# IceLab-X/FidelityFusion

Measured on AMD Instinct MI355X. Metric: GP NLML+Cholesky throughput (NxN fp64 GF/s, %MFMA-roofline) at N=16384, higher is better.
Workload: dtype f64; 1 GPU; headline: single-fidelity cigp NLML forward, ARD kernel, 1 block of N=16384 D=16 d=1 (BASELINE configs[2]); N=16384, D=16, d=1, blocks=1, blocks_in_flight_per_rank=1, parallelism=fidelity-shard x1 (LPT partition, one 8-byte all-reduce per step)

## Files before the change

### fidelityfusion_amd/csrc/gemm.hip

```cpp
#include <algorithm>

#include "ffgp_internal.h"

#define BK 16
#ifndef FFGP_PD_SMALL
#define FFGP_PD_SMALL 4
#endif

#ifdef FFGP_GEMM_TRACE
__device__ unsigned long long* ffgp_trace_buf = nullptr;
extern "C" int ffgp_debug_set_trace(void* p) {
  return hipMemcpyToSymbol(HIP_SYMBOL(ffgp_trace_buf), &p, sizeof(p)) == hipSuccess ? 0 : -1;
}
#define FFGP_TRACE(slot)                                                                            \
  do {                                                                                              \
    if (tid == 0 && ffgp_trace_buf) {                                                               \
      ffgp_trace_buf[(size_t)bid * 8 + (slot)] = __builtin_readcyclecounter();                      \
      if ((slot) == 0) {                                                                            \
        unsigned hwid = 0, xcc = 0;                                                                 \
        asm volatile("s_getreg_b32 %0, hwreg(HW_REG_HW_ID)" : "=s"(hwid));                          \
        asm volatile("s_getreg_b32 %0, hwreg(HW_REG_XCC_ID)" : "=s"(xcc));                          \
        ffgp_trace_buf[(size_t)bid * 8 + 6] = ((unsigned long long)xcc << 32) | hwid;               \
        ffgp_trace_buf[(size_t)bid * 8 + 7] = wall_clock64();                                       \
      }                                                                                             \
    }                                                                                               \
  } while (0)
#else
#define FFGP_TRACE(slot)
#endif

template <int TS>
struct Geo {
  static constexpr int WT = TS / 32;
  static constexpr int NLD = TS / 32;
  static constexpr int MNLD = TS + 16;
  static constexpr int OPBUF = 16 * (TS + 16);
};

__device__ __forceinline__ d2_t ld2_guard(const double* p, int rem, bool vec) {
  d2_t v = {0.0, 0.0};
  if (rem >= 2) {
    if (vec) {
      v = *reinterpret_cast<const d2_t*>(p);
    } else {
      v.x = p[0];
      v.y = p[1];
    }
  } else if (rem == 1) {
    v.x = p[0];
  }
  return v;
}

template <int OP, int TS, bool GUARD>
__device__ __forceinline__ void gload(const double* __restrict__ P, int ld, int r0, int R, int k0, int K, int tid,
                                      bool vec, d2_t (&v)[Geo<TS>::NLD]) {
#pragma unroll
  for (int i = 0; i < Geo<TS>::NLD; ++i) {
    const int idx = tid + 256 * i;
    d2_t z = {0.0, 0.0};
    if (OP == OP_KMAJOR) {
      const int row = idx >> 3, ch = idx & 7;
      const int gr = r0 + row, gk = k0 + ch * 2;
      if (GUARD)
        v[i] = (gr < R) ? ld2_guard(P + (size_t)gr * ld + gk, K - gk, vec) : z;
      else
        v[i] = *reinterpret_cast<const d2_t*>(P + (size_t)gr * ld + gk);
    } else {
      const int kk = idx / (TS / 2), c2 = idx % (TS / 2);
      const int gk = k0 + kk, gr = r0 + c2 * 2;
      if (GUARD)
        v[i] = (gk < K) ? ld2_guard(P + (size_t)gk * ld + gr, R - gr, vec) : z;
      else
        v[i] = *reinterpret_cast<const d2_t*>(P + (size_t)gk * ld + gr);
    }
  }
}

template <int OP, int TS>
__device__ __forceinline__ void sstore(double* s, int tid, const d2_t (&v)[Geo<TS>::NLD]) {
#pragma unroll
  for (int i = 0; i < Geo<TS>::NLD; ++i) {
    const int idx = tid + 256 * i;
    if (OP == OP_KMAJOR) {
      const int row = idx >> 3, ch = idx & 7;
      *reinterpret_cast<d2_t*>(s + row * 16 + ((ch ^ ((row >> 1) & 7)) << 1)) = v[i];
    } else {
      const int kk = idx / (TS / 2), c2 = idx % (TS / 2);
      *reinterpret_cast<d2_t*>(s + kk * Geo<TS>::MNLD + c2 * 2) = v[i];
    }
  }
}

template <int OP, int TS>
__device__ __forceinline__ void frag_offsets(int lane, int wbase, int (&off)[4]) {
#pragma unroll
  for (int kq = 0; kq < 4; ++kq) {
    if (OP == OP_KMAJOR) {
      const int row = wbase + (lane & 15);
      const int c0 = (lane >> 5) ^ ((lane & 15) >> 1);
      off[kq] = row * 16 + ((((kq << 1) ^ c0)) << 1) + ((lane >> 4) & 1);
    } else {
      off[kq] = (kq * 4 + (lane >> 4)) * Geo<TS>::MNLD + wbase + (lane & 15);
    }
  }
}

__device__ __forceinline__ void decode_tile(int t, int mode, int tiles_m, int tiles_n, int& ti, int& tj, const int GL = 3) {
  const int G = 1 << GL;
  if (mode == TILES_FULL) {
    const int band_sz = G * tiles_n;
    int r0 = 0;
    while (t >= band_sz) {
      t -= band_sz;
      r0 += G;
    }
    const int hgt = min(G, tiles_m - r0);
    if (hgt == G) {
      tj = t >> GL;
      ti = r0 + (t & (G - 1));
    } else {
      tj = t / hgt;
      ti = r0 + t % hgt;
    }
  } else {
    int r0 = 0, hgt = 0, fc = 0;
    while (true) {
      hgt = min(G, tiles_m - r0);
      fc = min(r0, tiles_n);
      const int nc = max(0, min(hgt, tiles_n - r0));
      const int cnt = hgt * fc + nc * hgt - nc * (nc - 1) / 2;
      if (t < cnt) break;
      t -= cnt;
      r0 += hgt;
    }
    if (t < hgt * fc) {
      if (hgt == G) {
        tj = t >> GL;
        ti = r0 + (t & (G - 1));
      } else {
        tj = t / hgt;
        ti = r0 + t % hgt;
      }
    } else {
      t -= hgt * fc;
      int c = 0;
      while (t >= hgt - c) {
        t -= hgt - c;
        ++c;
      }
      tj = r0 + c;
      ti = r0 + c + t;
    }
  }
}

template <int OP, int TS>
__device__ __forceinline__ void lane_byte_offsets(int ld, int tid, unsigned (&voff)[Geo<TS>::NLD]) {
#pragma unroll
  for (int i = 0; i < Geo<TS>::NLD; ++i) {
    const int idx = tid + 256 * i;
    if (OP == OP_KMAJOR) {
      const int row = idx >> 3, ch = idx & 7;
      voff[i] = (unsigned)(row * ld + ch * 2) * 8u;
    } else {
      const int kk = idx / (TS / 2), c2 = idx % (TS / 2);
      voff[i] = (unsigned)(kk * ld + c2 * 2) * 8u;
    }
  }
}

template <int TS>
__device__ __forceinline__ void gload_fast(const char* __restrict__ base, const unsigned (&voff)[Geo<TS>::NLD],
                                           d2_t (&v)[Geo<TS>::NLD]) {
#pragma unroll
  for (int i = 0; i < Geo<TS>::NLD; ++i) v[i] = *reinterpret_cast<const d2_t*>(base + voff[i]);
}

template <int OP, int TS>
constexpr int opbuf() { return OP == OP_KMAJOR ? TS * 16 : Geo<TS>::OPBUF; }

template <int OPA, int OPB, int TM, int TN, bool NEG, int PD>
__device__ __forceinline__ void gemm_tile_fast(const char* __restrict__ baseA, const char* __restrict__ baseB, size_t stepA,
                                               size_t stepB, char* __restrict__ baseC, size_t row4_bytes, unsigned voffC,
                                               bool load_c, double* smem, int nkt, int tid,
                                               const unsigned (&voffA)[Geo<TM>::NLD], const unsigned (&voffB)[Geo<TN>::NLD],
                                               const int (&offA)[4], const int (&offB)[4], int trace_bid) {
  constexpr int WM = Geo<TM>::WT, WN = Geo<TN>::WT;
  constexpr int BUFA = opbuf<OPA, TM>(), BUFB = opbuf<OPB, TN>(), STAGE = BUFA + BUFB;
  constexpr int subA = (OPA == OP_KMAJOR) ? 256 : 16;
  constexpr int subB = (OPB == OP_KMAJOR) ? 256 : 16;
  static_assert(PD == 1 || (PD & 1) == 0, "prefetch depth must be 1 or even (LDS stage parity is compile-time)");
  d2_t ra[PD][Geo<TM>::NLD], rb[PD][Geo<TN>::NLD];
#pragma unroll
  for (int s = 0; s < PD; ++s) {
    if (s < nkt) {
      gload_fast<TM>(baseA + s * stepA, voffA, ra[s]);
      gload_fast<TN>(baseB + s * stepB, voffB, rb[s]);
    }
  }
  d4_t acc[WM][WN];
  if (load_c) {
#pragma unroll
    for (int i = 0; i < WM; ++i)
#pragma unroll
      for (int r = 0; r < 4; ++r) {
        const char* rowb = baseC + (size_t)(i * 4 + r) * row4_bytes;
#pragma unroll
        for (int j = 0; j < WN; ++j) acc[i][j][r] = *reinterpret_cast<const double*>(rowb + voffC + j * 128);
      }
  } else {
#pragma unroll
    for (int i = 0; i < WM; ++i)
#pragma unroll
      for (int j = 0; j < WN; ++j) acc[i][j] = (d4_t){0.0, 0.0, 0.0, 0.0};
  }
  sstore<OPA, TM>(smem, tid, ra[0]);
  sstore<OPB, TN>(smem + BUFA, tid, rb[0]);
  __syncthreads();
#ifdef FFGP_GEMM_TRACE
  if (tid == 0 && ffgp_trace_buf) ffgp_trace_buf[(size_t)trace_bid * 8 + 1] = __builtin_readcyclecounter();
#endif
  baseA += (size_t)PD * stepA;
  baseB += (size_t)PD * stepB;
  for (int kt0 = 0; kt0 < nkt; kt0 += PD) {
#pragma unroll
    for (int u = 0; u < PD; ++u) {
      const int kt = kt0 + u;
      if (kt >= nkt) break;
      const int par = (PD == 1) ? (kt & 1) : (u & 1);
      const double* sA = smem + par * STAGE;
      const double* sB = sA + BUFA;
      if (kt + PD < nkt) {
        gload_fast<TM>(baseA, voffA, ra[u]);
        gload_fast<TN>(baseB, voffB, rb[u]);
        baseA += stepA;
        baseB += stepB;
      }
#pragma unroll
      for (int kq = 0; kq < 4; ++kq) {
        double a[WM], b[WN];
#pragma unroll
        for (int i = 0; i < WM; ++i) a[i] = sA[offA[kq] + i * subA];
#pragma unroll
        for (int j = 0; j < WN; ++j) b[j] = sB[offB[kq] + j * subB];
#pragma unroll
        for (int i = 0; i < WM; ++i)
#pragma unroll
          for (int j = 0; j < WN; ++j)
            acc[i][j] = __builtin_amdgcn_mfma_f64_16x16x4f64(a[i], b[j], acc[i][j], 0, 0, NEG ? 1 : 0);
      }
      if (kt + 1 < nkt) {
        double* dA = smem + (par ^ 1) * STAGE;
        sstore<OPA, TM>(dA, tid, ra[(u + 1) % PD]);
        sstore<OPB, TN>(dA + BUFA, tid, rb[(u + 1) % PD]);
      }
      __syncthreads();
    }
  }
#ifdef FFGP_GEMM_TRACE
  if (tid == 0 && ffgp_trace_buf) ffgp_trace_buf[(size_t)trace_bid * 8 + 2] = __builtin_readcyclecounter();
#endif
#pragma unroll
  for (int i = 0; i < WM; ++i)
#pragma unroll
    for (int r = 0; r < 4; ++r) {
      char* rowb = baseC + (size_t)(i * 4 + r) * row4_bytes;
#pragma unroll
      for (int j = 0; j < WN; ++j) *reinterpret_cast<double*>(rowb + voffC + j * 128) = acc[i][j][r];
    }
}

template <int OPA, int OPB, int TM, int TN, bool GUARD>
__device__ __forceinline__ void gemm_mainloop(const GemmArgs& p, const double* __restrict__ Ag, const double* __restrict__ Bg,
                                              double* smem, int m0, int n0, int kt0, int kt1, int tid,
                                              const int (&offA)[4], const int (&offB)[4],
                                              d4_t (&acc)[Geo<TM>::WT][Geo<TN>::WT]) {
  constexpr int WM = Geo<TM>::WT, WN = Geo<TN>::WT;
  constexpr int BUFA = opbuf<OPA, TM>(), BUFB = opbuf<OPB, TN>(), STAGE = BUFA + BUFB;
  constexpr int subA = (OPA == OP_KMAJOR) ? 256 : 16;
  constexpr int subB = (OPB == OP_KMAJOR) ? 256 : 16;
  d2_t ra[Geo<TM>::NLD], rb[Geo<TN>::NLD];
  gload<OPA, TM, GUARD>(Ag, p.lda, m0, p.m, kt0 * BK, p.k, tid, p.avec != 0, ra);
  gload<OPB, TN, GUARD>(Bg, p.ldb, n0, p.n, kt0 * BK, p.k, tid, p.bvec != 0, rb);
  sstore<OPA, TM>(smem, tid, ra);
  sstore<OPB, TN>(smem + BUFA, tid, rb);
  __syncthreads();
  for (int kt = kt0; kt < kt1; ++kt) {
    const int par = (kt - kt0) & 1;
    const double* sA = smem + par * STAGE;
    const double* sB = sA + BUFA;
    const bool more = (kt + 1 < kt1);
    if (more) {
      gload<OPA, TM, GUARD>(Ag, p.lda, m0, p.m, (kt + 1) * BK, p.k, tid, p.avec != 0, ra);
      gload<OPB, TN, GUARD>(Bg, p.ldb, n0, p.n, (kt + 1) * BK, p.k, tid, p.bvec != 0, rb);
    }
#pragma unroll
    for (int kq = 0; kq < 4; ++kq) {
      double a[WM], b[WN];
#pragma unroll
      for (int i = 0; i < WM; ++i) a[i] = sA[offA[kq] + i * subA];
#pragma unroll
      for (int j = 0; j < WN; ++j) b[j] = sB[offB[kq] + j * subB];
#pragma unroll
      for (int i = 0; i < WM; ++i)
#pragma unroll
        for (int j = 0; j < WN; ++j) acc[i][j] = __builtin_amdgcn_mfma_f64_16x16x4f64(a[i], b[j], acc[i][j], 0, 0, 0);
    }
    if (more) {
      double* dA = smem + (par ^ 1) * STAGE;
      sstore<OPA, TM>(dA, tid, ra);
      sstore<OPB, TN>(dA + BUFA, tid, rb);
    }
    __syncthreads();
  }
}

template <int OPA, int OPB, int MODE, int TM, int TN>
__device__ __forceinline__ void gemm_one_tile(const GemmArgs& p, const double* __restrict__ Ag, const double* __restrict__ Bg,
                                              double* __restrict__ Cg, double* smem, int ti, int tj, const int tid, const int bid) {
  constexpr int WM = Geo<TM>::WT, WN = Geo<TN>::WT;
  const int lane = tid & 63, wave = tid >> 6;
  const int wm = wave >> 1, wn = wave & 1;
  int offA[4], offB[4];
  frag_offsets<OPA, TM>(lane, wm * (TM / 2), offA);
  frag_offsets<OPB, TN>(lane, wn * (TN / 2), offB);
  const bool fast_ab = p.fast && p.avec && p.bvec;
  const int m0 = ti * TM, n0 = tj * TN;

  int kbeg = 0, kend = p.k;
  if (p.lo_i) kbeg = max(kbeg, ti * TM);
  if (p.lo_j) kbeg = max(kbeg, tj * TN);
  if (p.hi_i) kend = min(kend, (ti + 1) * TM);
  if (p.hi_j) kend = min(kend, (tj + 1) * TN);
  const int kt0 = kbeg / BK;
  const int kt1 = (kend + BK - 1) / BK;

  const bool interior = (m0 + TM <= p.m) && (n0 + TN <= p.n) && (kt1 * BK <= p.k) && p.avec && p.bvec;
  if constexpr (TM == 128 && TN == 128 && OPA == OP_KMAJOR && OPB == OP_KMAJOR) {
    if (p.pack && fast_ab && interior && kt0 == 0 && kt1 * BK == p.k && !(MODE == TILES_LOWER && m0 < n0 + TN)) return;
  }
  if (fast_ab && interior && kt0 < kt1 && !(MODE == TILES_LOWER && m0 < n0 + TN)) {
    const size_t k0 = (size_t)kt0 * BK;
    const char* bA = reinterpret_cast<const char*>(Ag) +
                     ((OPA == OP_KMAJOR) ? ((size_t)m0 * p.lda + k0) : (k0 * p.lda + m0)) * 8;
    const char* bB = reinterpret_cast<const char*>(Bg) +
                     ((OPB == OP_KMAJOR) ? ((size_t)n0 * p.ldb + k0) : (k0 * p.ldb + n0)) * 8;
    const size_t stepA = (OPA == OP_KMAJOR) ? (size_t)BK * 8 : (size_t)BK * p.lda * 8;
    const size_t stepB = (OPB == OP_KMAJOR) ? (size_t)BK * 8 : (size_t)BK * p.ldb * 8;
    char* bC = reinterpret_cast<char*>(Cg) + ((size_t)m0 * p.ldc + n0) * 8;
    const size_t row4 = (size_t)p.ldc * 32;
    constexpr int PD = (TM == 128) ? 1 : FFGP_PD_SMALL;
    unsigned voffA[Geo<TM>::NLD], voffB[Geo<TN>::NLD];
    lane_byte_offsets<OPA, TM>(p.lda, tid, voffA);
    lane_byte_offsets<OPB, TN>(p.ldb, tid, voffB);
    const unsigned voffC = (unsigned)((wm * (TM / 2) + (lane >> 4)) * p.ldc + wn * (TN / 2) + (lane & 15)) * 8u;
    if (p.alpha < 0.0)
      gemm_tile_fast<OPA, OPB, TM, TN, true, PD>(bA, bB, stepA, stepB, bC, row4, voffC, p.beta != 0.0, smem, kt1 - kt0, tid, voffA,
                                             voffB, offA, offB, bid);
    else
      gemm_tile_fast<OPA, OPB, TM, TN, false, PD>(bA, bB, stepA, stepB, bC, row4, voffC, p.beta != 0.0, smem, kt1 - kt0, tid, voffA,
                                              voffB, offA, offB, bid);
    FFGP_TRACE(3);
    return;
  }

  d4_t acc[WM][WN];
#pragma unroll
  for (int i = 0; i < WM; ++i)
#pragma unroll
    for (int j = 0; j < WN; ++j) acc[i][j] = (d4_t){0.0, 0.0, 0.0, 0.0};

  if (kt0 < kt1) {
    if (interior)
      gemm_mainloop<OPA, OPB, TM, TN, false>(p, Ag, Bg, smem, m0, n0, kt0, kt1, tid, offA, offB, acc);
    else
      gemm_mainloop<OPA, OPB, TM, TN, true>(p, Ag, Bg, smem, m0, n0, kt0, kt1, tid, offA, offB, acc);
  }

  FFGP_TRACE(2);
  const double alpha = p.alpha, beta = p.beta;
  const bool use_c = (beta != 0.0);
  const int rbase0 = m0 + wm * (TM / 2) + (lane >> 4);
  const int cbase = n0 + wn * (TN / 2) + (lane & 15);
  double cv[2][4][WN];
  auto load_group = [&](int i, double (&dst)[4][WN]) {
#pragma unroll
    for (int r = 0; r < 4; ++r) {
      const int rowc = min(rbase0 + i * 16 + 4 * r, p.m - 1);
#pragma unroll
      for (int j = 0; j < WN; ++j) {
        const int colc = min(cbase + j * 16, p.n - 1);
        dst[r][j] = Cg[(size_t)rowc * p.ldc + colc];
      }
    }
  };
  if (use_c) {
    load_group(0, cv[0]);
  } else {
#pragma unroll
    for (int b = 0; b < 2; ++b)
#pragma unroll
      for (int r = 0; r < 4; ++r)
#pragma unroll
        for (int j = 0; j < WN; ++j) cv[b][r][j] = 0.0;
  }
#pragma unroll
  for (int i = 0; i < WM; ++i) {
    if (use_c && i + 1 < WM) load_group(i + 1, cv[(i + 1) & 1]);
#pragma unroll
    for (int r = 0; r < 4; ++r) {
      const int row = rbase0 + i * 16 + 4 * r;
#pragma unroll
      for (int j = 0; j < WN; ++j) {
        const int col = cbase + j * 16;
        if (row < p.m && col < p.n && (MODE != TILES_LOWER || col <= row)) {
          Cg[(size_t)row * p.ldc + col] = alpha * acc[i][j][r] + beta * cv[i & 1][r][j];
        }
      }
    }
  }
  FFGP_TRACE(3);
}

template <int OPA, int OPB, int MODE, int TM, int TN>
__device__ __forceinline__ void gemm_block(const GemmArgs& p, const double* __restrict__ Ag, const double* __restrict__ Bg,
                                           double* __restrict__ Cg, double* smem, const int tid, const int bid) {
  FFGP_TRACE(0);
  if constexpr (TM == 128 && TN == 128) {
    if (bid >= p.split_at) {
      const int q = bid - p.split_at;
      int Ti, Tj;
      decode_tile(p.split_at + (q >> 2), MODE, p.tiles_m, p.tiles_n, Ti, Tj, p.band_log2);
      const int ti = __builtin_amdgcn_readfirstlane(2 * Ti + ((q >> 1) & 1));
      const int tj = __builtin_amdgcn_readfirstlane(2 * Tj + (q & 1));
      if (ti * 64 >= p.m || tj * 64 >= p.n || (MODE == TILES_LOWER && tj > ti)) return;
      gemm_one_tile<OPA, OPB, MODE, 64, 64>(p, Ag, Bg, Cg, smem, ti, tj, tid, bid);
      return;
    }
  }
  int t = bid;
  if (!(p.lo_i | p.lo_j | p.hi_i | p.hi_j)) {
    const int nwg = p.total_tiles;
    const int q = nwg >> 3, r = nwg & 7, xcd = bid & 7;
    t = (xcd < r ? xcd * (q + 1) : r * (q + 1) + (xcd - r) * q) + (bid >> 3);
  }
  int ti, tj;
  decode_tile(t, MODE, p.tiles_m, p.tiles_n, ti, tj, p.band_log2);
  ti = __builtin_amdgcn_readfirstlane(ti);
  tj = __builtin_amdgcn_readfirstlane(tj);
  gemm_one_tile<OPA, OPB, MODE, TM, TN>(p, Ag, Bg, Cg, smem, ti, tj, tid, bid);
}

template <int OPA, int OPB, int MODE, int TAG, int TM, int TN>
__global__ __launch_bounds__(256, 2) void ffgp_gemm_f64(GemmArgs p) {
  __shared__ __attribute__((aligned(16))) double smem[2 * (opbuf<OPA, TM>() + opbuf<OPB, TN>())];
  const int tid = threadIdx.x;
  if (p.pub_word && tid == 0 && blockIdx.x == 0 && blockIdx.y == 0 && blockIdx.z == 0)
    __hip_atomic_store(p.pub_word, p.pub_val, __ATOMIC_RELAXED, __HIP_MEMORY_SCOPE_SYSTEM);
  if (p.prio) __builtin_amdgcn_s_setprio(2);
  const double* __restrict__ Ag = p.A + (size_t)blockIdx.y * p.sA + (size_t)blockIdx.z * p.sA2;
  const double* __restrict__ Bg = p.B + (size_t)blockIdx.y * p.sB + (size_t)blockIdx.z * p.sB2;
  double* __restrict__ Cg = p.C + (size_t)blockIdx.y * p.sC + (size_t)blockIdx.z * p.sC2;
  gemm_block<OPA, OPB, MODE, TM, TN>(p, Ag, Bg, Cg, smem, tid, blockIdx.x);
}

template <int OPA, int OPB, int MODE, int TAG, int TM, int TN>
__global__ __launch_bounds__(256, 2) void ffgp_gemm_f64_rag(GemmRag q) {
  __shared__ __attribute__((aligned(16))) double smem[2 * (opbuf<OPA, TM>() + opbuf<OPB, TN>())];
  const int tid = threadIdx.x;
  const GemmRagMember& r = q.mem[blockIdx.y];
  if ((int)blockIdx.x >= r.grid) return;
  if (q.base.prio) __builtin_amdgcn_s_setprio(2);
  GemmArgs p = q.base;
  p.A = r.A; p.B = r.B; p.C = r.C;
  p.m = r.m; p.n = r.n; p.k = r.k;
  p.lda = r.lda; p.ldb = r.ldb; p.ldc = r.ldc;
  p.tiles_m = r.tiles_m; p.tiles_n = r.tiles_n; p.total_tiles = r.total_tiles;
  p.grid = r.grid; p.split_at = r.split_at;
  p.fast = r.fast; p.avec = r.avec; p.bvec = r.bvec;
  gemm_block<OPA, OPB, MODE, TM, TN>(p, p.A, p.B, p.C, smem, tid, blockIdx.x);
}

#define GEMM_BAND_LOG2 3
#define POLITE_PAD_KB 40
template <int OPA, int OPB, int MODE, int TAG, int TM, int TN>
static int launch_t(ffgp_handle* h, const GemmArgs& a) {
  if (a.pad_lds > 0)
    FFGP_HIP(hipFuncSetAttribute(reinterpret_cast<const void*>(&ffgp_gemm_f64<OPA, OPB, MODE, TAG, TM, TN>),
                                 hipFuncAttributeMaxDynamicSharedMemorySize, 64 * 1024));
  hipLaunchKernelGGL((ffgp_gemm_f64<OPA, OPB, MODE, TAG, TM, TN>), dim3(a.grid, a.batch, a.batch2), dim3(256), a.pad_lds, h->stream, a);
  return FFGP_OK;
}

template <int TS>
static int dispatch(ffgp_handle* h, int opa, int opb, int mode, int syrk_tag, const GemmArgs& a) {
  if (syrk_tag) {
    if (opa == OP_KMAJOR && opb == OP_KMAJOR && mode == TILES_LOWER) return launch_t<OP_KMAJOR, OP_KMAJOR, TILES_LOWER, 1, TS, TS>(h, a);
  } else if (mode == TILES_LOWER) {
    if (opa == OP_KMAJOR && opb == OP_KMAJOR) return launch_t<OP_KMAJOR, OP_KMAJOR, TILES_LOWER, 0, TS, TS>(h, a);
    if (opa == OP_MNMAJOR && opb == OP_MNMAJOR) return launch_t<OP_MNMAJOR, OP_MNMAJOR, TILES_LOWER, 0, TS, TS>(h, a);
  } else {
    if (opa == OP_KMAJOR && opb == OP_KMAJOR) return launch_t<OP_KMAJOR, OP_KMAJOR, TILES_FULL, 0, TS, TS>(h, a);
    if (opa == OP_KMAJOR && opb == OP_MNMAJOR) return launch_t<OP_KMAJOR, OP_MNMAJOR, TILES_FULL, 0, TS, TS>(h, a);
    if (opa == OP_MNMAJOR && opb == OP_MNMAJOR) return launch_t<OP_MNMAJOR, OP_MNMAJOR, TILES_FULL, 0, TS, TS>(h, a);
    if (opa == OP_MNMAJOR && opb == OP_KMAJOR) return launch_t<OP_MNMAJOR, OP_KMAJOR, TILES_FULL, 0, TS, TS>(h, a);
  }
  return FFGP_ERR_ARG;
}

static inline bool aligned16(const void* p) { return (reinterpret_cast<uintptr_t>(p) & 15) == 0; }

static int count_tiles(int mode, int m, int n, int tsm, int tsn, int& tm, int& tn) {
  tm = (m + tsm - 1) / tsm;
  tn = (n + tsn - 1) / tsn;
  if (mode != TILES_LOWER) return tm * tn;
  int total = 0;
  for (int ti = 0; ti < tm; ++ti) total += (ti + 1 < tn) ? ti + 1 : tn;
  return total;
}

__global__ __launch_bounds__(256) void ffgp_splitk_reduce(const double* __restrict__ P, int ldp, long sP, int parts, double* __restrict__ C,
                                                         int ldc, int m, int n, double beta) {
  const long e = (long)blockIdx.x * 256 + threadIdx.x;
  if (e >= (long)m * n) return;
  const int r = (int)(e / n), c = (int)(e - (long)r * n);
  double acc = 0.0;
  const double* p = P + (size_t)r * ldp + c;
  for (int s = 0; s < parts; ++s) acc += p[(size_t)s * sP];
  double* dst = C + (size_t)r * ldc + c;
  *dst = (beta != 0.0) ? acc + beta * *dst : acc;
}

static int ensure_skw(ffgp_handle* h, size_t bytes) {
  if (bytes <= h->skw_bytes) return FFGP_OK;
  if (h->skw) {
    hipStreamSynchronize(h->stream);
    if (h->aux) hipStreamSynchronize(h->aux);
    hipFree(h->skw);
  }
  h->skw = nullptr;
  h->skw_bytes = 0;
  const size_t gran = (size_t)16 << 20;
  const size_t want = (bytes + gran - 1) / gran * gran;
  if (hipMalloc(&h->skw, want) != hipSuccess) return FFGP_ERR_ALLOC;
  h->skw_bytes = want;
  ++h->alloc_epoch;
  return FFGP_OK;
}

struct SkinnyArgs {
  const double* A;
  const double* B;
  double* C;
  int m, n, k, lda, ldb, ldc, opb;
  int kc;
  long sP;
  int klo;
  int ldcj;
  double alpha, beta;
};

__device__ __forceinline__ double skinny_b(const SkinnyArgs& p, int kk, int j) {
  return (p.opb == OP_KMAJOR) ? p.B[(size_t)j * p.ldb + kk] : p.B[(size_t)kk * p.ldb + j];
}

template <int NC>
__global__ __launch_bounds__(256) void ffgp_skinny_kmajor(SkinnyArgs p) {
  const int lane = threadIdx.x & 63;
  const int row = blockIdx.x * 4 + (threadIdx.x >> 6);
  if (row >= p.m) return;
  const double* __restrict__ a = p.A + (size_t)row * p.lda;
  const int kbeg = blockIdx.y * p.kc, kend = min(p.k, kbeg + p.kc);
  double acc[NC];
#pragma unroll
  for (int j = 0; j < NC; ++j) acc[j] = 0.0;
#pragma unroll 4
  for (int k0 = max(kbeg, p.klo ? (row & ~127) : 0) + lane * 2; k0 < kend; k0 += 128) {
    const double a0 = a[k0];
    const bool two = k0 + 1 < kend;
    const double a1 = two ? a[k0 + 1] : 0.0;
#pragma unroll
    for (int j = 0; j < NC; ++j)
      if (j < p.n) {
        acc[j] = __builtin_fma(a0, skinny_b(p, k0, j), acc[j]);
        if (two) acc[j] = __builtin_fma(a1, skinny_b(p, k0 + 1, j), acc[j]);
      }
  }
#pragma unroll
  for (int j = 0; j < NC; ++j)
    for (int o = 32; o > 0; o >>= 1) acc[j] += __shfl_down(acc[j], o);
  if (lane == 0) {
#pragma unroll
    for (int j = 0; j < NC; ++j)
      if (j < p.n) {
        double* dst = p.C + blockIdx.y * p.sP + (size_t)row * p.ldc + (size_t)j * p.ldcj;
        *dst = (p.beta != 0.0) ? p.alpha * acc[j] + p.beta * *dst : p.alpha * acc[j];
      }
  }
}

template <int NC>
__global__ __launch_bounds__(512) void ffgp_skinny_mnmajor(SkinnyArgs p) {
  __shared__ double red[8][NC][64];
  const int lane = threadIdx.x & 63, w = threadIdx.x >> 6;
  const int row = blockIdx.x * 64 + lane;
  const int kbeg = blockIdx.y * p.kc, kend = min(p.k, kbeg + p.kc);
  const int k00 = max(kbeg, p.klo ? (int)blockIdx.x * 64 : 0);
  const int kchunk = (max(kend - k00, 0) + 7) / 8;
  const int kb = k00 + w * kchunk, ke = min(kend, kb + kchunk);
  double acc[NC];
#pragma unroll
  for (int j = 0; j < NC; ++j) acc[j] = 0.0;
  if (row < p.m) {
    const double* __restrict__ a = p.A + row;
#pragma unroll 8
    for (int kk = kb; kk < ke; ++kk) {
      const double av = a[(size_t)kk * p.lda];
#pragma unroll
      for (int j = 0; j < NC; ++j)
        if (j < p.n) acc[j] = __builtin_fma(av, skinny_b(p, kk, j), acc[j]);
    }
  }
#pragma unroll
  for (int j = 0; j < NC; ++j) red[w][j][lane] = acc[j];
  __syncthreads();
  if (w == 0 && row < p.m) {
#pragma unroll
    for (int j = 0; j < NC; ++j)
      if (j < p.n) {
        double s = 0.0;
#pragma unroll
        for (int q = 0; q < 8; ++q) s += red[q][j][lane];
        double* dst = p.C + blockIdx.y * p.sP + (size_t)row * p.ldc + (size_t)j * p.ldcj;
        *dst = (p.beta != 0.0) ? p.alpha * s + p.beta * *dst : p.alpha * s;
      }
  }
}

template <int NC>
static void launch_skinny(ffgp_handle* h, int opa, const SkinnyArgs& a, int parts = 1) {
  if (opa == OP_KMAJOR)
    hipLaunchKernelGGL(ffgp_skinny_kmajor<NC>, dim3((a.m + 3) / 4, parts), dim3(256), 0, h->stream, a);
  else
    hipLaunchKernelGGL(ffgp_skinny_mnmajor<NC>, dim3((a.m + 63) / 64, parts), dim3(512), 0, h->stream, a);
}

struct GemmPlan {
  GemmArgs a;
  int tsm, tsn;
  int syrk_tag;
};

static int gemm_plan(ffgp_handle* h, int opa, int opb, int mode, int syrk_tag, const double* A, int lda, const double* B, int ldb, double* C,
                     int ldc, int m, int n, int k, double alpha, double beta, int tri, int alias, int batch, long sA, long sB, long sC,
                     GemmPlan& pl) {
  GemmArgs& a = pl.a;
  a = GemmArgs();
  a.avec = (!(lda & 1) && aligned16(A)) ? 1 : 0;
  a.bvec = (!(ldb & 1) && aligned16(B)) ? 1 : 0;
  a.A = A; a.B = B; a.C = C;
  a.m = m; a.n = n; a.k = k;
  a.lda = lda; a.ldb = ldb; a.ldc = ldc;
  a.alpha = alpha; a.beta = beta;
  a.prio = (h->stream == h->aux && h->aux_prio) ? 1 : 0;
  a.batch2 = 1;
  a.sA2 = a.sB2 = a.sC2 = 0;
  const int dec_batch = (batch < 0) ? 1 : (batch > 1 ? batch : 1);
  if (batch < 0) batch = -batch;
  a.batch = batch > 1 ? batch : 1;
  a.sA = sA; a.sB = sB; a.sC = sC;
  if ((sA & 1) || (sB & 1)) a.avec = a.bvec = 0;
  a.lo_i = (tri & TRI_LO_I) ? 1 : 0;
  a.lo_j = (tri & TRI_LO_J) ? 1 : 0;
  a.hi_i = (tri & TRI_HI_I) ? 1 : 0;
  a.hi_j = (tri & TRI_HI_J) ? 1 : 0;
  int tsm = 128, tsn = 128;
  a.total_tiles = count_tiles(mode, m, n, 128, 128, a.tiles_m, a.tiles_n);
  int level = 0;
  if (h->force_ts == 64) level = 1;
  else if (h->force_ts == 32) level = 2;
  else if (h->force_ts == 0 && a.total_tiles * dec_batch < h->small_tile_threshold) level = 1;
  const bool kk = (opa == OP_KMAJOR && opb == OP_KMAJOR);
  if (level >= 1) {
    if (alias == 0 || (alias == ALIAS_A && n <= 64) || (alias == ALIAS_B && m <= 64)) {
      tsm = tsn = 64;
    } else if (alias == ALIAS_A && kk) {
      tsm = 64;
    }
    a.total_tiles = count_tiles(mode, m, n, tsm, tsn, a.tiles_m, a.tiles_n);
    if (h->force_ts == 0 && level == 1 && kk && dec_batch == 1 && tsm == 64 && a.total_tiles < h->tile32_threshold) level = 2;
    if (level == 2 && kk && tsm == 64 && dec_batch == 1 && alias != ALIAS_B) {
      tsm = 32;
      tsn = (alias == ALIAS_A) ? 128 : 32;
      a.total_tiles = count_tiles(mode, m, n, tsm, tsn, a.tiles_m, a.tiles_n);
    }
  }
  if ((alias == ALIAS_A && a.tiles_n != 1) || (alias == ALIAS_B && a.tiles_m != 1)) {
    fprintf(stderr, "[ffgp] gemm: in-place launch would be split across %d x %d tiles (alias %d)\n", a.tiles_m, a.tiles_n, alias);
    return FFGP_ERR_ARG;
  }
  a.fast = ((alpha == 1.0 || alpha == -1.0) && (beta == 0.0 || beta == 1.0) && (size_t)lda * 8 * 130 < 0xffffffffull &&
            (size_t)ldb * 8 * 130 < 0xffffffffull && (size_t)ldc * 8 * 130 < 0xffffffffull)
               ? 1 : 0;
  a.grid = a.total_tiles;
  a.split_at = 0x7fffffff;
  a.band_log2 = GEMM_BAND_LOG2;
  if (tsm == 128 && tsn == 128 && alias == 0 && dec_batch == 1 && h->force_ts == 0 && h->split_rem_max > 0 && a.total_tiles > 256) {
    const int rem = a.total_tiles % 256;
    if (rem > 0 && rem <= h->split_rem_max) {
      a.split_at = a.total_tiles - rem;
      a.total_tiles = a.split_at;
      a.grid = a.split_at + 4 * rem;
    }
  }
  a.pad_lds = 0;
  if (syrk_tag && tsm == 128 && h->lookahead && h->polite_m > 0 && m < h->polite_m && h->stream != h->aux) a.pad_lds = POLITE_PAD_KB * 1024;
  if (syrk_tag && tsm == 64 && tsn == 64 && h->polite64_active && h->polite64_pad_kb > 0 && h->stream != h->aux && dec_batch == 1 &&
      m - n <= 1024)
    a.pad_lds = h->polite64_pad_kb * 1024;
  if (syrk_tag && tsm == 32 && tsn == 32 && h->polite64_active && h->polite32_pad_kb > 0 && h->stream != h->aux && dec_batch == 1 && m - n <= 1024)
    a.pad_lds = h->polite32_pad_kb * 1024;
  a.pub_word = nullptr;
  a.pub_val = 0;
  if (h->ho_gdefer_slot >= 0 && h->ho_gdefer_stream == h->stream && h->ob_F <= 1) {
    a.pub_word = h->ho_mem + h->ho_gdefer_slot * 16;
    a.pub_val = h->ho_seq[h->ho_gdefer_slot];
    h->ho_launched[h->ho_gdefer_slot] = h->ho_seq[h->ho_gdefer_slot];
    h->ho_gdefer_slot = -1;
  }
  if (tsm != 128) syrk_tag = 0;
  pl.tsm = tsm; pl.tsn = tsn; pl.syrk_tag = syrk_tag;
  return FFGP_OK;
}

int ffgp_gemm_launch(ffgp_handle* h, int opa, int opb, int mode, int syrk_tag, const double* A, int lda, const double* B,
                     int ldb, double* C, int ldc, int m, int n, int k, double alpha, double beta, int tri, int alias, int batch,
                     long sA, long sB, long sC) {
  if (m <= 0 || n <= 0) return FFGP_OK;
  if (k <= 0) {
    return FFGP_ERR_ARG;
  }
  if (!A || !B || !C) return FFGP_ERR_ARG;
  if (mode == TILES_LOWER && m < n) return FFGP_ERR_ARG;
  if (alias == ALIAS_A && (n > 128 || mode != TILES_FULL)) return FFGP_ERR_ARG;
  if (alias == ALIAS_B && (m > 128 || mode != TILES_FULL)) return FFGP_ERR_ARG;
  const bool ob = h->ob_F > 1;
  long ob_sA = 0, ob_sB = 0, ob_sC = 0;
  if (ob) {
    auto stride_of = [&](const double* ptr, long& st) {
      for (int i = 0; i < h->ob_n; ++i)
        if (ptr >= h->ob_rng[i].lo && ptr < h->ob_rng[i].hi) { st = h->ob_rng[i].stride; return true; }
      return false;
    };
    if (!stride_of(A, ob_sA) || !stride_of(B, ob_sB) || !stride_of(C, ob_sC) || ((ob_sA | ob_sB | ob_sC) & 1) || alias != 0 || syrk_tag) {
      fprintf(stderr, "[ffgp] gemm: outer-batch launch with an operand outside the registered ranges\n");
      return FFGP_ERR_ARG;
    }
    if (tri == 0 || m <= 8 || n <= 8) {
      const int F = h->ob_F;
      h->ob_F = 0;
      int rc = FFGP_OK;
      for (int f = 0; f < F && rc == FFGP_OK; ++f)
        rc = ffgp_gemm_launch(h, opa, opb, mode, syrk_tag, A + (size_t)f * ob_sA, lda, B + (size_t)f * ob_sB, ldb, C + (size_t)f * ob_sC, ldc,
                              m, n, k, alpha, beta, tri, alias, batch, sA, sB, sC);
      h->ob_F = F;
      return rc;
    }
  }
  if (h->skinny_max_n > 0 && m <= h->skinny_max_n && m <= 8 && n > 8 && alias == 0 && (batch == 0 || batch == 1) && (tri == 0 || tri == TRI_LO_J) &&
      mode == TILES_FULL && !syrk_tag && h->stream != h->aux) {
// ... 262 lines not shown
```

Before: 52440 GF/s.

## Software-pipeline LDS fragment reads and split MFMA batches around global loads in GEMM

Restructures the fast GEMM tile main loop so the next k-quarter's LDS fragments are read ahead into double-buffered registers while the current MFMAs issue. The LDS store and the next global prefetch move into the middle of the MFMA stream, and only one barrier per k-tile remains, implemented as an explicit waitcnt plus s_barrier. The aim is to hide LDS and global-memory latency behind MFMA work. Separately, 32x32 tiles now get a higher minimum-workgroups launch bound (6), which raises occupancy at the cost of register pressure. Per-k-tile cycle tracing is also added, but only under the trace build flag.

```diff
diff --git a/fidelityfusion_amd/csrc/gemm.hip b/fidelityfusion_amd/csrc/gemm.hip
--- a/fidelityfusion_amd/csrc/gemm.hip
+++ b/fidelityfusion_amd/csrc/gemm.hip
@@ -12,9 +12,15 @@
 extern "C" int ffgp_debug_set_trace(void* p) {
   return hipMemcpyToSymbol(HIP_SYMBOL(ffgp_trace_buf), &p, sizeof(p)) == hipSuccess ? 0 : -1;
 }
+__device__ unsigned* ffgp_trace_seq = nullptr;
+__device__ unsigned ffgp_trace_cap = 0;
+extern "C" int ffgp_debug_set_trace_seq(void* counter, unsigned cap) {
+  return hipMemcpyToSymbol(HIP_SYMBOL(ffgp_trace_cap), &cap, sizeof(cap)) == hipSuccess &&
+                 hipMemcpyToSymbol(HIP_SYMBOL(ffgp_trace_seq), &counter, sizeof(counter)) == hipSuccess ? 0 : -1;
+}
 #define FFGP_TRACE(slot)                                                                            \
   do {                                                                                              \
-    if (tid == 0 && ffgp_trace_buf) {                                                               \
+    if (tid == 0 && ffgp_trace_buf && !ffgp_trace_seq) {                                            \
       ffgp_trace_buf[(size_t)bid * 8 + (slot)] = __builtin_readcyclecounter();                      \
       if ((slot) == 0) {                                                                            \
         unsigned hwid = 0, xcc = 0;                                                                 \
@@ -25,8 +31,17 @@
       }                                                                                             \
     }                                                                                               \
   } while (0)
+#define KT_STAMP(v)                          \
+  do {                                       \
+    if (KT_TRACE) {                          \
+      __builtin_amdgcn_sched_barrier(0);     \
+      v = __builtin_readcyclecounter();      \
+      __builtin_amdgcn_sched_barrier(0);     \
+    }                                        \
+  } while (0)
 #else
 #define FFGP_TRACE(slot)
+#define KT_STAMP(v)
 #endif
 
 template <int TS>
@@ -180,6 +195,22 @@
 template <int OP, int TS>
 constexpr int opbuf() { return OP == OP_KMAJOR ? TS * 16 : Geo<TS>::OPBUF; }
 
+#define GEMM_LDS_WAIT()                      \
+  do {                                       \
+    __builtin_amdgcn_sched_barrier(0);       \
+    asm volatile("" ::: "memory");           \
+    __builtin_amdgcn_s_waitcnt(0xc07f);      \
+  } while (0)
+#define GEMM_BARRIER() asm volatile("s_barrier" ::: "memory")
+
+template <int WM, int WN, int subA, int subB>
+__device__ __forceinline__ void frag_read(const double* sA, const double* sB, int oa, int ob, double (&a)[WM], double (&b)[WN]) {
+#pragma unroll
+  for (int i = 0; i < WM; ++i) a[i] = sA[oa + i * subA];
+#pragma unroll
+  for (int j = 0; j < WN; ++j) b[j] = sB[ob + j * subB];
+}
+
 template <int OPA, int OPB, int TM, int TN, bool NEG, int PD>
 __device__ __forceinline__ void gemm_tile_fast(const char* __restrict__ baseA, const char* __restrict__ baseB, size_t stepA,
                                                size_t stepB, char* __restrict__ baseC, size_t row4_bytes, unsigned voffC,
@@ -191,6 +222,9 @@
   constexpr int subA = (OPA == OP_KMAJOR) ? 256 : 16;
   constexpr int subB = (OPB == OP_KMAJOR) ? 256 : 16;
   static_assert(PD == 1 || (PD & 1) == 0, "prefetch depth must be 1 or even (LDS stage parity is compile-time)");
+  constexpr bool AHEAD = !(TM == 32 && TN == 128);
+  constexpr int HALF = (WM * WN + 1) / 2;
+  constexpr int U = (PD == 1) ? 2 : PD;
   d2_t ra[PD][Geo<TM>::NLD], rb[PD][Geo<TN>::NLD];
 #pragma unroll
   for (int s = 0; s < PD; ++s) {
@@ -199,6 +233,8 @@
       gload_fast<TN>(baseB + s * stepB, voffB, rb[s]);
     }
   }
+  baseA += (size_t)PD * stepA;
+  baseB += (size_t)PD * stepB;
   d4_t acc[WM][WN];
   if (load_c) {
 #pragma unroll
@@ -217,49 +253,109 @@
   }
   sstore<OPA, TM>(smem, tid, ra[0]);
   sstore<OPB, TN>(smem + BUFA, tid, rb[0]);
-  __syncthreads();
+  if (PD < nkt) {
+    gload_fast<TM>(baseA, voffA, ra[0]);
+    gload_fast<TN>(baseB, voffB, rb[0]);
+    baseA += stepA;
+    baseB += stepB;
+  }
+  GEMM_LDS_WAIT();
+  GEMM_BARRIER();
+  double fa[2][WM], fb[2][WN];
+  if (AHEAD) frag_read<WM, WN, subA, subB>(smem, smem + BUFA, offA[0], offB[0], fa[0], fb[0]);
 #ifdef FFGP_GEMM_TRACE
-  if (tid == 0 && ffgp_trace_buf) ffgp_trace_buf[(size_t)trace_bid * 8 + 1] = __builtin_readcyclecounter();
+  constexpr bool KT_TRACE = (TM == 128 && TN == 128);
+  size_t trow = (size_t)trace_bid;
+  bool ton = (tid == 0 && ffgp_trace_buf);
+  if (ton && ffgp_trace_seq) {
+    ton = false;
+    if (KT_TRACE) {
+      const unsigned r = atomicAdd(ffgp_trace_seq, 1u);
+      if (r < ffgp_trace_cap) {
+        unsigned hwid = 0, xcc = 0;
+        asm volatile("s_getreg_b32 %0, hwreg(HW_REG_HW_ID)" : "=s"(hwid));
+        asm volatile("s_getreg_b32 %0, hwreg(HW_REG_XCC_ID)" : "=s"(xcc));
+        ton = true;
+        trow = r;
+        ffgp_trace_buf[trow * 8 + 6] = ((unsigned long long)gridDim.x << 40) | ((unsigned long long)(xcc & 0xf) << 32) | hwid;
+        ffgp_trace_buf[trow * 8 + 7] = wall_clock64();
+      }
+    }
+  }
+  if (ton) ffgp_trace_buf[trow * 8 + 1] = __builtin_readcyclecounter();
+  unsigned long long t_l = 0, t_b = 0, t_x = 0, t_m = 0, t_w0 = 0, t_w1 = 0;
+  unsigned kt_first = 0, kt_vm = 0, kt_bar = 0, kt_lds = 0;
 #endif
-  baseA += (size_t)PD * stepA;
-  baseB += (size_t)PD * stepB;
-  for (int kt0 = 0; kt0 < nkt; kt0 += PD) {
-#pragma unroll
-    for (int u = 0; u < PD; ++u) {
+  for (int kt0 = 0; kt0 < nkt; kt0 += U) {
+#pragma unroll
+    for (int u = 0; u < U; ++u) {
       const int kt = kt0 + u;
       if (kt >= nkt) break;
-      const int par = (PD == 1) ? (kt & 1) : (u & 1);
-      const double* sA = smem + par * STAGE;
-      const double* sB = sA + BUFA;
-      if (kt + PD < nkt) {
-        gload_fast<TM>(baseA, voffA, ra[u]);
-        gload_fast<TN>(baseB, voffB, rb[u]);
-        baseA += stepA;
-        baseB += stepB;
-      }
+      const double* sCur = smem + (u & 1) * STAGE;
+      double* sNxt = smem + ((u & 1) ^ 1) * STAGE;
+      const bool more = (kt + 1 < nkt);
 #pragma unroll
       for (int kq = 0; kq < 4; ++kq) {
-        double a[WM], b[WN];
-#pragma unroll
-        for (int i = 0; i < WM; ++i) a[i] = sA[offA[kq] + i * subA];
-#pragma unroll
-        for (int j = 0; j < WN; ++j) b[j] = sB[offB[kq] + j * subB];
-#pragma unroll
-        for (int i = 0; i < WM; ++i)
-#pragma unroll
-          for (int j = 0; j < WN; ++j)
-            acc[i][j] = __builtin_amdgcn_mfma_f64_16x16x4f64(a[i], b[j], acc[i][j], 0, 0, NEG ? 1 : 0);
-      }
-      if (kt + 1 < nkt) {
-        double* dA = smem + (par ^ 1) * STAGE;
-        sstore<OPA, TM>(dA, tid, ra[(u + 1) % PD]);
-        sstore<OPB, TN>(dA + BUFA, tid, rb[(u + 1) % PD]);
-      }
-      __syncthreads();
-    }
-  }
+        const int sn = AHEAD ? ((kq + 1) & 1) : 0;
+        if (!AHEAD) {
+          frag_read<WM, WN, subA, subB>(sCur, sCur + BUFA, offA[kq], offB[kq], fa[0], fb[0]);
+        } else if (kq < 3) {
+          frag_read<WM, WN, subA, subB>(sCur, sCur + BUFA, offA[kq + 1], offB[kq + 1], fa[sn], fb[sn]);
+        } else {
+          KT_STAMP(t_l);
+          GEMM_LDS_WAIT();
+          if (more) {
+            KT_STAMP(t_b);
+            GEMM_BARRIER();
+            KT_STAMP(t_x);
+            frag_read<WM, WN, subA, subB>(sNxt, sNxt + BUFA, offA[0], offB[0], fa[sn], fb[sn]);
+          }
+        }
+        if (AHEAD) __builtin_amdgcn_sched_barrier(0);
+        if (kq == 3 && more) KT_STAMP(t_m);
+        const int sc = AHEAD ? (kq & 1) : 0;
+#pragma unroll
+        for (int e = 0; e < HALF; ++e)
+          acc[e / WN][e % WN] = __builtin_amdgcn_mfma_f64_16x16x4f64(fa[sc][e / WN], fb[sc][e % WN], acc[e / WN][e % WN], 0, 0, NEG ? 1 : 0);
+        if (kq == 1 && more) {
+          const int sl = (u + 1) % PD;
+          KT_STAMP(t_w0);
+          sstore<OPA, TM>(sNxt, tid, ra[sl]);
+          sstore<OPB, TN>(sNxt + BUFA, tid, rb[sl]);
+          KT_STAMP(t_w1);
+          if (kt + 1 + PD < nkt) {
+            gload_fast<TM>(baseA, voffA, ra[sl]);
+            gload_fast<TN>(baseB, voffB, rb[sl]);
+            baseA += stepA;
+            baseB += stepB;
+          }
+        }
+#pragma unroll
+        for (int e = HALF; e < WM * WN; ++e)
+          acc[e / WN][e % WN] = __builtin_amdgcn_mfma_f64_16x16x4f64(fa[sc][e / WN], fb[sc][e % WN], acc[e / WN][e % WN], 0, 0, NEG ? 1 : 0);
+        if (!AHEAD && kq == 3 && more) {
+          GEMM_LDS_WAIT();
+          GEMM_BARRIER();
+        }
+      }
 #ifdef FFGP_GEMM_TRACE
-  if (tid == 0 && ffgp_trace_buf) ffgp_trace_buf[(size_t)trace_bid * 8 + 2] = __builtin_readcyclecounter();
+      if (KT_TRACE && more) {
+        kt_first += (unsigned)(t_m - t_x);
+        kt_vm += (unsigned)(t_w1 - t_w0);
+        kt_bar += (unsigned)(t_x - t_b);
+        kt_lds += (unsigned)(t_b - t_l);
+      }
+#endif
+    }
+  }
+#ifdef FFGP_GEMM_TRACE
+  if (ton) {
+    ffgp_trace_buf[trow * 8 + 2] = __builtin_readcyclecounter();
+    if (KT_TRACE) {
+      ffgp_trace_buf[trow * 8 + 4] = ((unsigned long long)kt_bar << 32) | kt_first;
+      ffgp_trace_buf[trow * 8 + 5] = ((unsigned long long)(nkt < 255 ? nkt : 255) << 56) | ((unsigned long long)(kt_lds & 0xffffffu) << 32) | kt_vm;
+    }
+  }
 #endif
 #pragma unroll
   for (int i = 0; i < WM; ++i)
@@ -452,8 +548,10 @@
   gemm_one_tile<OPA, OPB, MODE, TM, TN>(p, Ag, Bg, Cg, smem, ti, tj, tid, bid);
 }
 
+#define GEMM_MIN_WG(TM, TN) (((TM) == 32 && (TN) == 32) ? 6 : 2)
+
 template <int OPA, int OPB, int MODE, int TAG, int TM, int TN>
-__global__ __launch_bounds__(256, 2) void ffgp_gemm_f64(GemmArgs p) {
+__global__ __launch_bounds__(256, (GEMM_MIN_WG(TM, TN))) void ffgp_gemm_f64(GemmArgs p) {
   __shared__ __attribute__((aligned(16))) double smem[2 * (opbuf<OPA, TM>() + opbuf<OPB, TN>())];
   const int tid = threadIdx.x;
   if (p.pub_word && tid == 0 && blockIdx.x == 0 && blockIdx.y == 0 && blockIdx.z == 0)
@@ -466,7 +564,7 @@
 }
 
 template <int OPA, int OPB, int MODE, int TAG, int TM, int TN>
-__global__ __launch_bounds__(256, 2) void ffgp_gemm_f64_rag(GemmRag q) {
+__global__ __launch_bounds__(256, (GEMM_MIN_WG(TM, TN))) void ffgp_gemm_f64_rag(GemmRag q) {
   __shared__ __attribute__((aligned(16))) double smem[2 * (opbuf<OPA, TM>() + opbuf<OPB, TN>())];
   const int tid = threadIdx.x;
   const GemmRagMember& r = q.mem[blockIdx.y];
```

Measured after the change: 54020 GF/s (median of 6 runs). +3.0%, better.

## Add software-pipelined 128x128 fast GEMM tile with buffer loads and sched barriers

Applied to the files above, without the earlier changes.

Adds a dedicated 128x128 interior GEMM tile path. It uses raw buffer loads and double-buffered LDS stages, and interleaves LDS reads for the next k-quarter with the MFMA batch for the current one. Scheduling barriers pin that order so LDS latency and global loads overlap with fp64 MFMA work. This targets the trailing-update GEMMs that dominate the Cholesky. The cost is register pressure from the doubled fragment registers, and the pinned schedule may constrain the compiler.

```diff
diff --git a/fidelityfusion_amd/csrc/gemm.hip b/fidelityfusion_amd/csrc/gemm.hip
--- a/fidelityfusion_amd/csrc/gemm.hip
+++ b/fidelityfusion_amd/csrc/gemm.hip
@@ -1,6 +1,7 @@
 #include <algorithm>
 
 #include "ffgp_internal.h"
+#include "diag_block.h"
 
 #define BK 16
 #ifndef FFGP_PD_SMALL
@@ -268,6 +269,115 @@
       char* rowb = baseC + (size_t)(i * 4 + r) * row4_bytes;
 #pragma unroll
       for (int j = 0; j < WN; ++j) *reinterpret_cast<double*>(rowb + voffC + j * 128) = acc[i][j][r];
+    }
+}
+
+typedef unsigned gemm_v4u __attribute__((ext_vector_type(4)));
+__device__ __forceinline__ __amdgpu_buffer_rsrc_t gemm_rsrc(const char* base) {
+  return __builtin_amdgcn_make_buffer_rsrc(const_cast<char*>(base), 0, 0xffffffff, 0x00020000);
+}
+template <int TS>
+__device__ __forceinline__ void gload_buf(__amdgpu_buffer_rsrc_t r, const unsigned (&voff)[Geo<TS>::NLD], d2_t (&v)[Geo<TS>::NLD]) {
+#pragma unroll
+  for (int i = 0; i < Geo<TS>::NLD; ++i) v[i] = __builtin_bit_cast(d2_t, (gemm_v4u)__builtin_amdgcn_raw_buffer_load_b128(r, (int)voff[i], 0, 0));
+}
+
+template <int OPA, int OPB, bool NEG>
+__device__ __forceinline__ void gemm_tile_fast128(const char* __restrict__ baseA, const char* __restrict__ baseB, size_t stepA, size_t stepB,
+                                                  char* __restrict__ baseC, size_t row4_bytes, unsigned voffC, bool load_c, double* smem,
+                                                  int nkt, int tid, const unsigned (&voffA)[4], const unsigned (&voffB)[4],
+                                                  const int (&offA)[4], const int (&offB)[4], int trace_bid) {
+  constexpr int TS = 128, W = 4;
+  constexpr int BUFA = opbuf<OPA, TS>(), BUFB = opbuf<OPB, TS>(), STAGE = BUFA + BUFB;
+  constexpr int subA = (OPA == OP_KMAJOR) ? 256 : 16;
+  constexpr int subB = (OPB == OP_KMAJOR) ? 256 : 16;
+#define GEMM_PIN() __builtin_amdgcn_sched_barrier(0)
+#define GEMM_READ(st, kq, a, b)                                         \
+  do {                                                                  \
+    _Pragma("unroll") for (int i = 0; i < W; ++i) a[i] = (st)[offA[kq] + i * subA];        \
+    _Pragma("unroll") for (int j = 0; j < W; ++j) b[j] = (st)[BUFA + offB[kq] + j * subB]; \
+    GEMM_PIN();                                                         \
+  } while (0)
+#define GEMM_MFMA(a, b)                                                 \
+  do {                                                                  \
+    _Pragma("unroll") for (int i = 0; i < W; ++i)                       \
+      _Pragma("unroll") for (int j = 0; j < W; ++j)                     \
+        acc[i][j] = __builtin_amdgcn_mfma_f64_16x16x4f64(a[i], b[j], acc[i][j], 0, 0, NEG ? 1 : 0);  \
+    GEMM_PIN();                                                         \
+  } while (0)
+  d2_t ra[4], rb[4];
+  gload_buf<TS>(gemm_rsrc(baseA), voffA, ra);
+  gload_buf<TS>(gemm_rsrc(baseB), voffB, rb);
+  d4_t acc[W][W];
+  if (load_c) {
+#pragma unroll
+    for (int i = 0; i < W; ++i)
+#pragma unroll
+      for (int r = 0; r < 4; ++r) {
+        const char* rowb = baseC + (size_t)(i * 4 + r) * row4_bytes;
+#pragma unroll
+        for (int j = 0; j < W; ++j) acc[i][j][r] = *reinterpret_cast<const double*>(rowb + voffC + j * 128);
+      }
+  } else {
+#pragma unroll
+    for (int i = 0; i < W; ++i)
+#pragma unroll
+      for (int j = 0; j < W; ++j) acc[i][j] = (d4_t){0.0, 0.0, 0.0, 0.0};
+  }
+  sstore<OPA, TS>(smem, tid, ra);
+  sstore<OPB, TS>(smem + BUFA, tid, rb);
+  LDS_BARRIER();
+#ifdef FFGP_GEMM_TRACE
+  if (tid == 0 && ffgp_trace_buf) ffgp_trace_buf[(size_t)trace_bid * 8 + 1] = __builtin_readcyclecounter();
+#endif
+  double xa[W], xb[W], ya[W], yb[W];
+  GEMM_PIN();
+  GEMM_READ(smem, 0, xa, xb);
+  for (int kt = 0; kt + 1 < nkt; ++kt) {
+    const double* sS = smem + (kt & 1) * STAGE;
+    double* sN = smem + ((kt & 1) ^ 1) * STAGE;
+    baseA += stepA;
+    baseB += stepB;
+    gload_buf<TS>(gemm_rsrc(baseA), voffA, ra);
+    gload_buf<TS>(gemm_rsrc(baseB), voffB, rb);
+    GEMM_PIN();
+    GEMM_READ(sS, 1, ya, yb);
+    GEMM_MFMA(xa, xb);
+    GEMM_READ(sS, 2, xa, xb);
+    GEMM_MFMA(ya, yb);
+    sstore<OPA, TS>(sN, tid, ra);
+    sstore<OPB, TS>(sN + BUFA, tid, rb);
+    GEMM_PIN();
+    GEMM_READ(sS, 3, ya, yb);
+    GEMM_MFMA(xa, xb);
+    LDS_BARRIER();
+    GEMM_PIN();
+    GEMM_READ(sN, 0, xa, xb);
+    GEMM_MFMA(ya, yb);
+  }
+  {
+    const double* sS = smem + ((nkt - 1) & 1) * STAGE;
+    GEMM_READ(sS, 1, ya, yb);
+    GEMM_MFMA(xa, xb);
+    GEMM_READ(sS, 2, xa, xb);
+    GEMM_MFMA(ya, yb);
+    GEMM_READ(sS, 3, ya, yb);
+    GEMM_MFMA(xa, xb);
+    GEMM_MFMA(ya, yb);
+  }
+#undef GEMM_PIN
+#undef GEMM_READ
+#undef GEMM_MFMA
+#ifdef FFGP_GEMM_TRACE
+  if (tid == 0 && ffgp_trace_buf) ffgp_trace_buf[(size_t)trace_bid * 8 + 2] = __builtin_readcyclecounter();
+#endif
+#pragma unroll
+  for (int i = 0; i < W; ++i)
+#pragma unroll
+    for (int r = 0; r < 4; ++r) {
+      char* rowb = baseC + (size_t)(i * 4 + r) * row4_bytes;
+#pragma unroll
+      for (int j = 0; j < W; ++j) *reinterpret_cast<double*>(rowb + voffC + j * 128) = acc[i][j][r];
     }
 }
 
@@ -355,7 +465,12 @@
     lane_byte_offsets<OPA, TM>(p.lda, tid, voffA);
     lane_byte_offsets<OPB, TN>(p.ldb, tid, voffB);
     const unsigned voffC = (unsigned)((wm * (TM / 2) + (lane >> 4)) * p.ldc + wn * (TN / 2) + (lane & 15)) * 8u;
-    if (p.alpha < 0.0)
+    if constexpr (TM == 128 && TN == 128) {
+      if (p.alpha < 0.0)
+        gemm_tile_fast128<OPA, OPB, true>(bA, bB, stepA, stepB, bC, row4, voffC, p.beta != 0.0, smem, kt1 - kt0, tid, voffA, voffB, offA, offB, bid);
+      else
+        gemm_tile_fast128<OPA, OPB, false>(bA, bB, stepA, stepB, bC, row4, voffC, p.beta != 0.0, smem, kt1 - kt0, tid, voffA, voffB, offA, offB, bid);
+    } else if (p.alpha < 0.0)
       gemm_tile_fast<OPA, OPB, TM, TN, true, PD>(bA, bB, stepA, stepB, bC, row4, voffC, p.beta != 0.0, smem, kt1 - kt0, tid, voffA,
                                              voffB, offA, offB, bid);
     else
```

Result: faster. 52470 GF/s before, 53510 GF/s after, median of 6 (+2.0%).
